# microsoft/Nova

Hardware: NVIDIA H100
Metric: MSM throughput (2^20 BN254 scalar*G1/s) (higher is better)
Workload: dtype u32 limbs (256-bit prime-field / curve integers)

## Files before the change

### nova_b200/csrc/field.cuh

```cuda
#pragma once
#include <cstdint>
#include "field_constants.cuh"

#if defined(__CUDACC__)
#define NOVA_HD __host__ __device__ __forceinline__
#define NOVA_D __device__ __forceinline__
#else
#define NOVA_HD inline
#define NOVA_D inline
#endif

namespace nova {

struct alignas(16) fe_t {
  uint32_t l[8];
};


template <int OFF, bool CIN, int N>
NOVA_HD void chain_mad(uint32_t (&X)[N], uint32_t x0, uint32_t x1, uint32_t x2, uint32_t x3,
                       uint32_t y, uint32_t ca = 0, uint32_t cb = 0) {
  static_assert(OFF + 8 < N, "accumulator too short");
#ifdef __CUDA_ARCH__
  if constexpr (CIN) {
    asm("{\n\t"
        ".reg .u32 t;\n\t"
        "add.cc.u32 t, %14, %15;\n\t"
        "madc.lo.cc.u32 %0, %9, %13, %0;\n\t"
        "madc.hi.cc.u32 %1, %9, %13, %1;\n\t"
        "madc.lo.cc.u32 %2, %10, %13, %2;\n\t"
        "madc.hi.cc.u32 %3, %10, %13, %3;\n\t"
        "madc.lo.cc.u32 %4, %11, %13, %4;\n\t"
        "madc.hi.cc.u32 %5, %11, %13, %5;\n\t"
        "madc.lo.cc.u32 %6, %12, %13, %6;\n\t"
        "madc.hi.cc.u32 %7, %12, %13, %7;\n\t"
        "addc.u32 %8, %8, 0;\n\t"
        "}"
        : "+r"(X[OFF + 0]), "+r"(X[OFF + 1]), "+r"(X[OFF + 2]), "+r"(X[OFF + 3]),
          "+r"(X[OFF + 4]), "+r"(X[OFF + 5]), "+r"(X[OFF + 6]), "+r"(X[OFF + 7]),
          "+r"(X[OFF + 8])
        : "r"(x0), "r"(x1), "r"(x2), "r"(x3), "r"(y), "r"(ca), "r"(cb));
  } else {
    asm("mad.lo.cc.u32 %0, %9, %13, %0;\n\t"
        "madc.hi.cc.u32 %1, %9, %13, %1;\n\t"
        "madc.lo.cc.u32 %2, %10, %13, %2;\n\t"
        "madc.hi.cc.u32 %3, %10, %13, %3;\n\t"
        "madc.lo.cc.u32 %4, %11, %13, %4;\n\t"
        "madc.hi.cc.u32 %5, %11, %13, %5;\n\t"
        "madc.lo.cc.u32 %6, %12, %13, %6;\n\t"
        "madc.hi.cc.u32 %7, %12, %13, %7;\n\t"
        "addc.u32 %8, %8, 0;"
        : "+r"(X[OFF + 0]), "+r"(X[OFF + 1]), "+r"(X[OFF + 2]), "+r"(X[OFF + 3]),
          "+r"(X[OFF + 4]), "+r"(X[OFF + 5]), "+r"(X[OFF + 6]), "+r"(X[OFF + 7]),
          "+r"(X[OFF + 8])
        : "r"(x0), "r"(x1), "r"(x2), "r"(x3), "r"(y));
  }
#else
  uint64_t cf = CIN ? (((uint64_t)ca + cb) >> 32) : 0;
  const uint32_t xs[4] = {x0, x1, x2, x3};
  for (int k = 0; k < 4; k++) {
    uint64_t prod = (uint64_t)xs[k] * y;
    uint64_t t = (uint64_t)X[OFF + 2 * k] + (uint32_t)prod + cf;
    X[OFF + 2 * k] = (uint32_t)t;
    cf = t >> 32;
    t = (uint64_t)X[OFF + 2 * k + 1] + (prod >> 32) + cf;
    X[OFF + 2 * k + 1] = (uint32_t)t;
    cf = t >> 32;
  }
  X[OFF + 8] += (uint32_t)cf;
#endif
}

NOVA_HD void add8(uint32_t (&r)[8], const uint32_t (&a)[8], const uint32_t (&b)[8]) {
#ifdef __CUDA_ARCH__
  asm("add.cc.u32 %0, %8, %16;\n\t"
      "addc.cc.u32 %1, %9, %17;\n\t"
      "addc.cc.u32 %2, %10, %18;\n\t"
      "addc.cc.u32 %3, %11, %19;\n\t"
      "addc.cc.u32 %4, %12, %20;\n\t"
      "addc.cc.u32 %5, %13, %21;\n\t"
      "addc.cc.u32 %6, %14, %22;\n\t"
      "addc.u32 %7, %15, %23;"
      : "=r"(r[0]), "=r"(r[1]), "=r"(r[2]), "=r"(r[3]), "=r"(r[4]), "=r"(r[5]), "=r"(r[6]),
        "=r"(r[7])
      : "r"(a[0]), "r"(a[1]), "r"(a[2]), "r"(a[3]), "r"(a[4]), "r"(a[5]), "r"(a[6]), "r"(a[7]),
        "r"(b[0]), "r"(b[1]), "r"(b[2]), "r"(b[3]), "r"(b[4]), "r"(b[5]), "r"(b[6]), "r"(b[7]));
#else
  uint64_t c = 0;
  for (int i = 0; i < 8; i++) {
    uint64_t t = (uint64_t)a[i] + b[i] + c;
    r[i] = (uint32_t)t;
    c = t >> 32;
  }
#endif
}

NOVA_HD void add8_cin(uint32_t (&r)[8], const uint32_t* a, const uint32_t* b, uint32_t ca,
                      uint32_t cb) {
#ifdef __CUDA_ARCH__
  asm("{\n\t"
      ".reg .u32 t;\n\t"
      "add.cc.u32 t, %24, %25;\n\t"
      "addc.cc.u32 %0, %8, %16;\n\t"
      "addc.cc.u32 %1, %9, %17;\n\t"
      "addc.cc.u32 %2, %10, %18;\n\t"
      "addc.cc.u32 %3, %11, %19;\n\t"
      "addc.cc.u32 %4, %12, %20;\n\t"
      "addc.cc.u32 %5, %13, %21;\n\t"
      "addc.cc.u32 %6, %14, %22;\n\t"
      "addc.u32 %7, %15, %23;\n\t"
      "}"
      : "=r"(r[0]), "=r"(r[1]), "=r"(r[2]), "=r"(r[3]), "=r"(r[4]), "=r"(r[5]), "=r"(r[6]),
        "=r"(r[7])
      : "r"(a[0]), "r"(a[1]), "r"(a[2]), "r"(a[3]), "r"(a[4]), "r"(a[5]), "r"(a[6]), "r"(a[7]),
        "r"(b[0]), "r"(b[1]), "r"(b[2]), "r"(b[3]), "r"(b[4]), "r"(b[5]), "r"(b[6]), "r"(b[7]),
        "r"(ca), "r"(cb));
#else
  uint64_t c = ((uint64_t)ca + cb) >> 32;
  for (int i = 0; i < 8; i++) {
    uint64_t t = (uint64_t)a[i] + b[i] + c;
    r[i] = (uint32_t)t;
    c = t >> 32;
  }
#endif
}

NOVA_HD uint32_t sub8(uint32_t (&r)[8], const uint32_t (&a)[8], const uint32_t (&b)[8]) {
  uint32_t borrow;
#ifdef __CUDA_ARCH__
  asm("sub.cc.u32 %0, %9, %17;\n\t"
      "subc.cc.u32 %1, %10, %18;\n\t"
      "subc.cc.u32 %2, %11, %19;\n\t"
      "subc.cc.u32 %3, %12, %20;\n\t"
      "subc.cc.u32 %4, %13, %21;\n\t"
      "subc.cc.u32 %5, %14, %22;\n\t"
      "subc.cc.u32 %6, %15, %23;\n\t"
      "subc.cc.u32 %7, %16, %24;\n\t"
      "subc.u32 %8, 0, 0;"
      : "=r"(r[0]), "=r"(r[1]), "=r"(r[2]), "=r"(r[3]), "=r"(r[4]), "=r"(r[5]), "=r"(r[6]),
        "=r"(r[7]), "=r"(borrow)
      : "r"(a[0]), "r"(a[1]), "r"(a[2]), "r"(a[3]), "r"(a[4]), "r"(a[5]), "r"(a[6]), "r"(a[7]),
        "r"(b[0]), "r"(b[1]), "r"(b[2]), "r"(b[3]), "r"(b[4]), "r"(b[5]), "r"(b[6]), "r"(b[7]));
#else
  uint64_t c = 0;
  for (int i = 0; i < 8; i++) {
    uint64_t t = (uint64_t)a[i] - b[i] - c;
    r[i] = (uint32_t)t;
    c = (t >> 32) & 1;
  }
  borrow = c ? 0xffffffffu : 0u;
#endif
  return borrow;
}

template <class F>
NOVA_HD void load_p(uint32_t (&p)[8]) {
#pragma unroll
  for (int i = 0; i < 8; i++) p[i] = F::p(i);
}


template <class F>
NOVA_HD fe_t fe_zero() {
  fe_t r;
#pragma unroll
  for (int i = 0; i < 8; i++) r.l[i] = 0;
  return r;
}

template <class F>
NOVA_HD fe_t fe_one() {
  fe_t r;
#pragma unroll
  for (int i = 0; i < 8; i++) r.l[i] = F::r(i);
  return r;
}

NOVA_HD bool fe_is_zero(const fe_t& a) {
  return (a.l[0] | a.l[1] | a.l[2] | a.l[3] | a.l[4] | a.l[5] | a.l[6] | a.l[7]) == 0;
}

NOVA_HD bool fe_eq(const fe_t& a, const fe_t& b) {
  return ((a.l[0] ^ b.l[0]) | (a.l[1] ^ b.l[1]) | (a.l[2] ^ b.l[2]) | (a.l[3] ^ b.l[3]) |
          (a.l[4] ^ b.l[4]) | (a.l[5] ^ b.l[5]) | (a.l[6] ^ b.l[6]) | (a.l[7] ^ b.l[7])) == 0;
}

template <class F>
NOVA_HD bool fe_is_canonical(const fe_t& a) {
  uint32_t p[8], t[8];
  load_p<F>(p);
  return sub8(t, a.l, p) != 0;
}

template <class F>
NOVA_HD void fe_reduce_once(uint32_t (&r)[8]) {
  uint32_t p[8], t[8];
  load_p<F>(p);
  uint32_t borrow = sub8(t, r, p);
#pragma unroll
  for (int i = 0; i < 8; i++) r[i] = borrow ? r[i] : t[i];
}

template <class F>
NOVA_HD fe_t fe_add(const fe_t& a, const fe_t& b) {
  fe_t r;
  add8(r.l, a.l, b.l);
  fe_reduce_once<F>(r.l);
  return r;
}

template <class F>
NOVA_HD fe_t fe_sub(const fe_t& a, const fe_t& b) {
  fe_t r;
  uint32_t p[8], t[8];
  load_p<F>(p);
  uint32_t borrow = sub8(r.l, a.l, b.l);
  add8(t, r.l, p);
#pragma unroll
  for (int i = 0; i < 8; i++) r.l[i] = borrow ? t[i] : r.l[i];
  return r;
}

template <class F>
NOVA_HD fe_t fe_neg(const fe_t& a) {
  fe_t z = fe_zero<F>();
  return fe_is_zero(a) ? z : fe_sub<F>(z, a);
}

template <class F>
NOVA_HD fe_t fe_dbl(const fe_t& a) {
  return fe_add<F>(a, a);
}

template <class F, int I>
NOVA_HD void mont_round(uint32_t (&E)[17], uint32_t (&O)[17], const fe_t& a, uint32_t bi) {
  if constexpr ((I & 1) == 0) {
    if constexpr (I == 0)
      chain_mad<I, false>(E, a.l[0], a.l[2], a.l[4], a.l[6], bi);
    else
      chain_mad<I, true>(E, a.l[0], a.l[2], a.l[4], a.l[6], bi, E[I - 1], O[I - 1]);
    chain_mad<I + 1, false>(O, a.l[1], a.l[3], a.l[5], a.l[7], bi);
    uint32_t m = (E[I] + O[I]) * F::INV;
    chain_mad<I, false>(E, F::p(0), F::p(2), F::p(4), F::p(6), m);
    chain_mad<I + 1, false>(O, F::p(1), F::p(3), F::p(5), F::p(7), m);
  } else {
    chain_mad<I, true>(O, a.l[0], a.l[2], a.l[4], a.l[6], bi, E[I - 1], O[I - 1]);
    chain_mad<I + 1, false>(E, a.l[1], a.l[3], a.l[5], a.l[7], bi);
    uint32_t m = (E[I] + O[I]) * F::INV;
    chain_mad<I, false>(O, F::p(0), F::p(2), F::p(4), F::p(6), m);
    chain_mad<I + 1, false>(E, F::p(1), F::p(3), F::p(5), F::p(7), m);
  }
}

template <class F>
NOVA_HD fe_t fe_mul_chain(const fe_t& a, const fe_t& b) {
  uint32_t E[17], O[17];
#pragma unroll
  for (int i = 0; i < 17; i++) E[i] = O[i] = 0;
  mont_round<F, 0>(E, O, a, b.l[0]);
  mont_round<F, 1>(E, O, a, b.l[1]);
  mont_round<F, 2>(E, O, a, b.l[2]);
  mont_round<F, 3>(E, O, a, b.l[3]);
  mont_round<F, 4>(E, O, a, b.l[4]);
  mont_round<F, 5>(E, O, a, b.l[5]);
  mont_round<F, 6>(E, O, a, b.l[6]);
  mont_round<F, 7>(E, O, a, b.l[7]);
  fe_t r;
  add8_cin(r.l, &E[8], &O[8], E[7], O[7]);
  fe_reduce_once<F>(r.l);
  return r;
}

template <class F, int I>
NOVA_HD void mont_round2(uint32_t (&E)[17], uint32_t (&O)[17], const fe_t& a, uint32_t bi, const fe_t& c,
                         uint32_t di) {
  if constexpr ((I & 1) == 0) {
    if constexpr (I == 0)
      chain_mad<I, false>(E, a.l[0], a.l[2], a.l[4], a.l[6], bi);
    else
      chain_mad<I, true>(E, a.l[0], a.l[2], a.l[4], a.l[6], bi, E[I - 1], O[I - 1]);
    chain_mad<I + 1, false>(O, a.l[1], a.l[3], a.l[5], a.l[7], bi);
    chain_mad<I, false>(E, c.l[0], c.l[2], c.l[4], c.l[6], di);
    chain_mad<I + 1, false>(O, c.l[1], c.l[3], c.l[5], c.l[7], di);
    uint32_t m = (E[I] + O[I]) * F::INV;
    chain_mad<I, false>(E, F::p(0), F::p(2), F::p(4), F::p(6), m);
    chain_mad<I + 1, false>(O, F::p(1), F::p(3), F::p(5), F::p(7), m);
  } else {
    chain_mad<I, true>(O, a.l[0], a.l[2], a.l[4], a.l[6], bi, E[I - 1], O[I - 1]);
    chain_mad<I + 1, false>(E, a.l[1], a.l[3], a.l[5], a.l[7], bi);
    chain_mad<I, false>(O, c.l[0], c.l[2], c.l[4], c.l[6], di);
    chain_mad<I + 1, false>(E, c.l[1], c.l[3], c.l[5], c.l[7], di);
    uint32_t m = (E[I] + O[I]) * F::INV;
    chain_mad<I, false>(O, F::p(0), F::p(2), F::p(4), F::p(6), m);
    chain_mad<I + 1, false>(E, F::p(1), F::p(3), F::p(5), F::p(7), m);
  }
}

template <class F>
NOVA_HD fe_t fe_mul2_add(const fe_t& a, const fe_t& b, const fe_t& c, const fe_t& d) {
  uint32_t E[17], O[17];
#pragma unroll
  for (int i = 0; i < 17; i++) E[i] = O[i] = 0;
  mont_round2<F, 0>(E, O, a, b.l[0], c, d.l[0]);
  mont_round2<F, 1>(E, O, a, b.l[1], c, d.l[1]);
  mont_round2<F, 2>(E, O, a, b.l[2], c, d.l[2]);
  mont_round2<F, 3>(E, O, a, b.l[3], c, d.l[3]);
  mont_round2<F, 4>(E, O, a, b.l[4], c, d.l[4]);
  mont_round2<F, 5>(E, O, a, b.l[5], c, d.l[5]);
  mont_round2<F, 6>(E, O, a, b.l[6], c, d.l[6]);
  mont_round2<F, 7>(E, O, a, b.l[7], c, d.l[7]);
  fe_t r;
  add8_cin(r.l, &E[8], &O[8], E[7], O[7]);
  fe_reduce_once<F>(r.l);
  return r;
}

NOVA_HD void mad_cs(uint32_t& lo, uint32_t& hi, uint32_t& k, uint32_t x, uint32_t y) {
#ifdef __CUDA_ARCH__
  asm("mad.lo.cc.u32 %0, %3, %4, %0;\n\t"
      "madc.hi.cc.u32 %1, %3, %4, %1;\n\t"
      "addc.u32 %2, %2, 0;"
      : "+r"(lo), "+r"(hi), "+r"(k)
      : "r"(x), "r"(y));
#else
  uint64_t acc = ((uint64_t)hi << 32) | lo;
  uint64_t prod = (uint64_t)x * y;
  uint64_t s = acc + prod;
  k += s < prod ? 1u : 0u;
  lo = (uint32_t)s;
  hi = (uint32_t)(s >> 32);
#endif
}

NOVA_HD void retire_cs(uint32_t& k_next, uint32_t e, uint32_t o, uint32_t kz) {
#ifdef __CUDA_ARCH__
  [[maybe_unused]] uint32_t t;
  asm("add.cc.u32 %1, %2, %3;\n\t"
      "addc.u32 %0, %0, %4;"
      : "+r"(k_next), "=r"(t)
      : "r"(e), "r"(o), "r"(kz));
#else
  k_next += (uint32_t)(((uint64_t)e + o) >> 32) + kz;
#endif
}

template <class F, int I>
NOVA_HD void mont_round_cs(uint32_t (&E)[16], uint32_t (&O)[16], uint32_t (&K)[17], const fe_t& a,
                           uint32_t bi) {
  uint32_t(&A)[16] = (I & 1) ? O : E;
  uint32_t(&B)[16] = (I & 1) ? E : O;
  mad_cs(A[I + 0], A[I + 1], K[I + 2], a.l[0], bi);
  mad_cs(B[I + 1], B[I + 2], K[I + 3], a.l[1], bi);
  mad_cs(A[I + 2], A[I + 3], K[I + 4], a.l[2], bi);
  mad_cs(B[I + 3], B[I + 4], K[I + 5], a.l[3], bi);
  mad_cs(A[I + 4], A[I + 5], K[I + 6], a.l[4], bi);
  mad_cs(B[I + 5], B[I + 6], K[I + 7], a.l[5], bi);
  mad_cs(A[I + 6], A[I + 7], K[I + 8], a.l[6], bi);
  mad_cs(B[I + 7], B[I + 8], K[I + 9], a.l[7], bi);
  uint32_t m = (E[I] + O[I] + K[I]) * F::INV;
  mad_cs(A[I + 0], A[I + 1], K[I + 2], F::p(0), m);
  mad_cs(B[I + 1], B[I + 2], K[I + 3], F::p(1), m);
  mad_cs(A[I + 2], A[I + 3], K[I + 4], F::p(2), m);
  mad_cs(B[I + 3], B[I + 4], K[I + 5], F::p(3), m);
  mad_cs(A[I + 4], A[I + 5], K[I + 6], F::p(4), m);
  mad_cs(B[I + 5], B[I + 6], K[I + 7], F::p(5), m);
  mad_cs(A[I + 6], A[I + 7], K[I + 8], F::p(6), m);
  mad_cs(B[I + 7], B[I + 8], K[I + 9], F::p(7), m);
  retire_cs(K[I + 1], E[I], O[I], K[I] ? 1u : 0u);
}

template <class F>
NOVA_HD fe_t fe_mul_cs(const fe_t& a, const fe_t& b) {
  uint32_t E[16], O[16], K[17];
#pragma unroll
  for (int i = 0; i < 16; i++) E[i] = O[i] = K[i] = 0;
  K[16] = 0;
  mont_round_cs<F, 0>(E, O, K, a, b.l[0]);
  mont_round_cs<F, 1>(E, O, K, a, b.l[1]);
  mont_round_cs<F, 2>(E, O, K, a, b.l[2]);
  mont_round_cs<F, 3>(E, O, K, a, b.l[3]);
  mont_round_cs<F, 4>(E, O, K, a, b.l[4]);
  mont_round_cs<F, 5>(E, O, K, a, b.l[5]);
  mont_round_cs<F, 6>(E, O, K, a, b.l[6]);
  mont_round_cs<F, 7>(E, O, K, a, b.l[7]);
  uint32_t hiE[8], hiO[8], hiK[8], t[8];
#pragma unroll
  for (int i = 0; i < 8; i++) {
    hiE[i] = E[8 + i];
    hiO[i] = O[8 + i];
    hiK[i] = K[8 + i];
  }
  fe_t r;
  add8(t, hiE, hiO);
  add8(r.l, t, hiK);
  fe_reduce_once<F>(r.l);
  return r;
}

template <class F>
NOVA_HD fe_t fe_mul(const fe_t& a, const fe_t& b) {
#ifdef NOVA_MUL_CS
  return fe_mul_cs<F>(a, b);
#else
  return fe_mul_chain<F>(a, b);
#endif
}


template <int OFF, int NP, int N>
NOVA_HD void chain_mad_n(uint32_t (&X)[N], uint32_t x0, uint32_t x1, uint32_t x2, uint32_t x3, uint32_t y) {
  static_assert(NP >= 1 && NP <= 4 && OFF + 2 * NP < N, "chain does not fit the accumulator");
#ifdef __CUDA_ARCH__
  if constexpr (NP == 1) {
    asm("mad.lo.cc.u32 %0, %3, %4, %0;\n\t"
        "madc.hi.cc.u32 %1, %3, %4, %1;\n\t"
        "addc.u32 %2, %2, 0;"
        : "+r"(X[OFF + 0]), "+r"(X[OFF + 1]), "+r"(X[OFF + 2])
        : "r"(x0), "r"(y));
  } else if constexpr (NP == 2) {
    asm("mad.lo.cc.u32 %0, %5, %7, %0;\n\t"
        "madc.hi.cc.u32 %1, %5, %7, %1;\n\t"
        "madc.lo.cc.u32 %2, %6, %7, %2;\n\t"
        "madc.hi.cc.u32 %3, %6, %7, %3;\n\t"
        "addc.u32 %4, %4, 0;"
        : "+r"(X[OFF + 0]), "+r"(X[OFF + 1]), "+r"(X[OFF + 2]), "+r"(X[OFF + 3]), "+r"(X[OFF + 4])
        : "r"(x0), "r"(x1), "r"(y));
  } else if constexpr (NP == 3) {
    asm("mad.lo.cc.u32 %0, %7, %10, %0;\n\t"
        "madc.hi.cc.u32 %1, %7, %10, %1;\n\t"
        "madc.lo.cc.u32 %2, %8, %10, %2;\n\t"
        "madc.hi.cc.u32 %3, %8, %10, %3;\n\t"
        "madc.lo.cc.u32 %4, %9, %10, %4;\n\t"
        "madc.hi.cc.u32 %5, %9, %10, %5;\n\t"
        "addc.u32 %6, %6, 0;"
        : "+r"(X[OFF + 0]), "+r"(X[OFF + 1]), "+r"(X[OFF + 2]), "+r"(X[OFF + 3]), "+r"(X[OFF + 4]),
          "+r"(X[OFF + 5]), "+r"(X[OFF + 6])
        : "r"(x0), "r"(x1), "r"(x2), "r"(y));
  } else {
    asm("mad.lo.cc.u32 %0, %9, %13, %0;\n\t"
        "madc.hi.cc.u32 %1, %9, %13, %1;\n\t"
        "madc.lo.cc.u32 %2, %10, %13, %2;\n\t"
        "madc.hi.cc.u32 %3, %10, %13, %3;\n\t"
        "madc.lo.cc.u32 %4, %11, %13, %4;\n\t"
        "madc.hi.cc.u32 %5, %11, %13, %5;\n\t"
        "madc.lo.cc.u32 %6, %12, %13, %6;\n\t"
        "madc.hi.cc.u32 %7, %12, %13, %7;\n\t"
        "addc.u32 %8, %8, 0;"
        : "+r"(X[OFF + 0]), "+r"(X[OFF + 1]), "+r"(X[OFF + 2]), "+r"(X[OFF + 3]), "+r"(X[OFF + 4]),
          "+r"(X[OFF + 5]), "+r"(X[OFF + 6]), "+r"(X[OFF + 7]), "+r"(X[OFF + 8])
        : "r"(x0), "r"(x1), "r"(x2), "r"(x3), "r"(y));
  }
#else
  const uint32_t xs[4] = {x0, x1, x2, x3};
  uint64_t cf = 0;
  for (int k = 0; k < NP; k++) {
    uint64_t prod = (uint64_t)xs[k] * y;
    uint64_t t = (uint64_t)X[OFF + 2 * k] + (uint32_t)prod + cf;
    X[OFF + 2 * k] = (uint32_t)t;
    cf = t >> 32;
    t = (uint64_t)X[OFF + 2 * k + 1] + (prod >> 32) + cf;
    X[OFF + 2 * k + 1] = (uint32_t)t;
    cf = t >> 32;
  }
  X[OFF + 2 * NP] += (uint32_t)cf;
#endif
}

NOVA_HD void chain_sqr_diag(uint32_t (&X)[17], const fe_t& a) {
#ifdef __CUDA_ARCH__
  asm("mad.lo.cc.u32 %0, %17, %17, %0;\n\t"
      "madc.hi.cc.u32 %1, %17, %17, %1;\n\t"
      "madc.lo.cc.u32 %2, %18, %18, %2;\n\t"
      "madc.hi.cc.u32 %3, %18, %18, %3;\n\t"
      "madc.lo.cc.u32 %4, %19, %19, %4;\n\t"
      "madc.hi.cc.u32 %5, %19, %19, %5;\n\t"
      "madc.lo.cc.u32 %6, %20, %20, %6;\n\t"
      "madc.hi.cc.u32 %7, %20, %20, %7;\n\t"
      "madc.lo.cc.u32 %8, %21, %21, %8;\n\t"
      "madc.hi.cc.u32 %9, %21, %21, %9;\n\t"
      "madc.lo.cc.u32 %10, %22, %22, %10;\n\t"
      "madc.hi.cc.u32 %11, %22, %22, %11;\n\t"
      "madc.lo.cc.u32 %12, %23, %23, %12;\n\t"
      "madc.hi.cc.u32 %13, %23, %23, %13;\n\t"
      "madc.lo.cc.u32 %14, %24, %24, %14;\n\t"
      "madc.hi.cc.u32 %15, %24, %24, %15;\n\t"
      "addc.u32 %16, %16, 0;"
      : "+r"(X[0]), "+r"(X[1]), "+r"(X[2]), "+r"(X[3]), "+r"(X[4]), "+r"(X[5]), "+r"(X[6]), "+r"(X[7]),
        "+r"(X[8]), "+r"(X[9]), "+r"(X[10]), "+r"(X[11]), "+r"(X[12]), "+r"(X[13]), "+r"(X[14]), "+r"(X[15]),
        "+r"(X[16])
      : "r"(a.l[0]), "r"(a.l[1]), "r"(a.l[2]), "r"(a.l[3]), "r"(a.l[4]), "r"(a.l[5]), "r"(a.l[6]), "r"(a.l[7]));
#else
  uint64_t cf = 0;
  for (int k = 0; k < 8; k++) {
    uint64_t prod = (uint64_t)a.l[k] * a.l[k];
    uint64_t t = (uint64_t)X[2 * k] + (uint32_t)prod + cf;
    X[2 * k] = (uint32_t)t;
    cf = t >> 32;
    t = (uint64_t)X[2 * k + 1] + (prod >> 32) + cf;
    X[2 * k + 1] = (uint32_t)t;
    cf = t >> 32;
  }
  X[16] += (uint32_t)cf;
#endif
}

template <int J>
NOVA_HD void sqr_cross(uint32_t (&E)[17], uint32_t (&O)[17], const fe_t& a) {
  constexpr int SAME0 = J & 1;
  constexpr int NSAME = J / 2;
  constexpr int OTH0 = 1 - (J & 1);
  constexpr int NOTH = (J + 1) / 2;
  const uint32_t y = a.l[J];
  auto limb = [&](int i) { return i < 8 ? a.l[i] : 0u; };
  if constexpr (NSAME > 0)
    chain_mad_n<SAME0 + J, NSAME>(E, limb(SAME0), limb(SAME0 + 2), limb(SAME0 + 4), limb(SAME0 + 6), y);
  if constexpr (NOTH > 0)
    chain_mad_n<OTH0 + J, NOTH>(O, limb(OTH0), limb(OTH0 + 2), limb(OTH0 + 4), limb(OTH0 + 6), y);
}

template <class F, int I>
NOVA_HD void mont_reduce_round(uint32_t (&E)[17], uint32_t (&O)[17]) {
  uint32_t c = 0;
  if constexpr (I > 0) c = (uint32_t)(((uint64_t)E[I - 1] + O[I - 1]) >> 32);
  const uint32_t m = (E[I] + O[I] + c) * F::INV;
  if constexpr ((I & 1) == 0) {
    if constexpr (I == 0)
      chain_mad<I, false>(E, F::p(0), F::p(2), F::p(4), F::p(6), m);
    else
      chain_mad<I, true>(E, F::p(0), F::p(2), F::p(4), F::p(6), m, E[I - 1], O[I - 1]);
    chain_mad<I + 1, false>(O, F::p(1), F::p(3), F::p(5), F::p(7), m);
  } else {
    chain_mad<I, true>(O, F::p(0), F::p(2), F::p(4), F::p(6), m, E[I - 1], O[I - 1]);
    chain_mad<I + 1, false>(E, F::p(1), F::p(3), F::p(5), F::p(7), m);
  }
}

template <class F>
NOVA_HD fe_t fe_sqr_dedicated(const fe_t& a) {
  uint32_t E[17], O[17];
#pragma unroll
  for (int i = 0; i < 17; i++) E[i] = O[i] = 0;
  sqr_cross<1>(E, O, a);
  sqr_cross<2>(E, O, a);
  sqr_cross<3>(E, O, a);
  sqr_cross<4>(E, O, a);
  sqr_cross<5>(E, O, a);
  sqr_cross<6>(E, O, a);
  sqr_cross<7>(E, O, a);
#pragma unroll
  for (int i = 16; i > 0; i--) {
    E[i] = (E[i] << 1) | (E[i - 1] >> 31);
    O[i] = (O[i] << 1) | (O[i - 1] >> 31);
  }
  E[0] <<= 1;
  O[0] <<= 1;
  chain_sqr_diag(E, a);
  uint32_t hiE[8], hiO[8], lo[8], hi[8];
#pragma unroll
  for (int i = 0; i < 8; i++) {
    hiE[i] = E[8 + i];
    hiO[i] = O[8 + i];
    E[8 + i] = 0;
    O[8 + i] = 0;
  }
  E[16] = O[16] = 0;
  mont_reduce_round<F, 0>(E, O);
  mont_reduce_round<F, 1>(E, O);
  mont_reduce_round<F, 2>(E, O);
  mont_reduce_round<F, 3>(E, O);
  mont_reduce_round<F, 4>(E, O);
  mont_reduce_round<F, 5>(E, O);
  mont_reduce_round<F, 6>(E, O);
  mont_reduce_round<F, 7>(E, O);
  add8_cin(lo, &E[8], &O[8], E[7], O[7]);
  add8(hi, hiE, hiO);
  fe_t r;
  add8(r.l, hi, lo);
  fe_reduce_once<F>(r.l);
  return r;
}

template <class F>
NOVA_HD fe_t fe_sqr(const fe_t& a) {
#if defined(NOVA_SQR_DEDICATED) && !defined(NOVA_MUL_CS)
  return fe_sqr_dedicated<F>(a);
#else
  return fe_mul<F>(a, a);
#endif
}

template <class F>
NOVA_HD fe_t fe_from_mont(const fe_t& a) {
  fe_t one;
#pragma unroll
  for (int i = 0; i < 8; i++) one.l[i] = (i == 0);
  return fe_mul<F>(a, one);
}

template <class F>
NOVA_HD fe_t fe_to_mont(const fe_t& a) {
  fe_t r2;
#pragma unroll
  for (int i = 0; i < 8; i++) r2.l[i] = F::r2(i);
  return fe_mul<F>(a, r2);
}

template <class F>
NOVA_HD fe_t fe_inv(const fe_t& a) {
  uint32_t e[8];
  uint32_t bw = 2;
#pragma unroll
  for (int i = 0; i < 8; i++) {
    uint32_t pi = F::p(i);
    e[i] = pi - bw;
    bw = (pi < bw) ? 1u : 0u;
  }
  fe_t acc = fe_one<F>();
  for (int i = 255; i >= 0; i--) {
    acc = fe_sqr<F>(acc);
    if ((e[i >> 5] >> (i & 31)) & 1) acc = fe_mul<F>(acc, a);
  }
  return acc;
}

#if defined(__CUDACC__)
NOVA_D fe_t fe_load(const void* base, size_t idx) {
  const uint4* p = reinterpret_cast<const uint4*>(base) + 2 * idx;
  uint4 lo = __ldg(p), hi = __ldg(p + 1);
  fe_t r;
  r.l[0] = lo.x; r.l[1] = lo.y; r.l[2] = lo.z; r.l[3] = lo.w;
  r.l[4] = hi.x; r.l[5] = hi.y; r.l[6] = hi.z; r.l[7] = hi.w;
  return r;
}
NOVA_D fe_t fe_load_rw(const void* base, size_t idx) {
  const uint4* p = reinterpret_cast<const uint4*>(base) + 2 * idx;
  uint4 lo = p[0], hi = p[1];
  fe_t r;
  r.l[0] = lo.x; r.l[1] = lo.y; r.l[2] = lo.z; r.l[3] = lo.w;
  r.l[4] = hi.x; r.l[5] = hi.y; r.l[6] = hi.z; r.l[7] = hi.w;
  return r;
}
NOVA_D void fe_store(void* base, size_t idx, const fe_t& a) {
  uint4* p = reinterpret_cast<uint4*>(base) + 2 * idx;
  p[0] = make_uint4(a.l[0], a.l[1], a.l[2], a.l[3]);
  p[1] = make_uint4(a.l[4], a.l[5], a.l[6], a.l[7]);
}
#elif defined(NOVA_SIMT_HOST)
inline fe_t fe_load(const void* base, size_t idx) { return reinterpret_cast<const fe_t*>(base)[idx]; }
inline fe_t fe_load_rw(const void* base, size_t idx) { return reinterpret_cast<const fe_t*>(base)[idx]; }
inline void fe_store(void* base, size_t idx, const fe_t& a) { reinterpret_cast<fe_t*>(base)[idx] = a; }
#endif

}
```

### nova_b200/csrc/msm_sort.cuh

```cuda
#pragma once
#if !defined(NOVA_SIMT_HOST)
#include <cuda_runtime.h>
#endif
#include <cstddef>
#include <cstdint>
#include "field.cuh"

namespace nova {

constexpr uint32_t NO_KEY = 0xFFFFFFFFu;

constexpr int SORT_THREADS = 256;
constexpr int SORT_WARPS = SORT_THREADS / 32;
constexpr int SORT_ITEMS = 16;
constexpr int SORT_TILE = SORT_THREADS * SORT_ITEMS;
constexpr int SORT_RADIX_MAX = 8;
constexpr int SORT_BINS = 1 << SORT_RADIX_MAX;
constexpr int SORT_PASSES_MAX = 4;
constexpr int SORT_CTL_WORDS = SORT_PASSES_MAX * SORT_BINS + SORT_PASSES_MAX;
constexpr unsigned SORT_HIST_BLOCKS = 1024;
constexpr int SORT_LOOK_WINDOW = 4;
constexpr int SORT_MIN_BLOCKS = 3;
static_assert(SORT_BINS == SORT_THREADS, "the per-bin steps run one bin per thread");

struct sort_plan {
  int passes;
  int bits;
};

inline sort_plan make_sort_plan(uint64_t K) {
  int kb = 1;
  while (kb < 32 && ((uint64_t)1 << kb) < K) kb++;
  sort_plan sp;
  sp.passes = (kb + SORT_RADIX_MAX - 1) / SORT_RADIX_MAX;
  sp.bits = (kb + sp.passes - 1) / sp.passes;
  return sp;
}

struct sort_args {
  uint32_t n;
  uint32_t count;
  int W, G;
  uint32_t B;
  uint32_t n_ck;
  uint32_t base_offset;
  uint32_t blind_i;
  uint32_t h_index;
  sort_plan sp;
};

NOVA_D void sort_hist_clear(uint32_t* sh ) {
  for (int i = threadIdx.x; i < SORT_PASSES_MAX * SORT_BINS; i += blockDim.x) sh[i] = 0;
  __syncthreads();
}

NOVA_D void sort_hist_count(uint32_t* sh, uint32_t key, const sort_plan sp) {
  const bool live = key != NO_KEY;
  const unsigned live_mask = __ballot_sync(0xFFFFFFFFu, live);
  if (live_mask == 0) return;
  const unsigned lane = threadIdx.x & 31u, leader = (unsigned)(__ffs(live_mask) - 1);
  const uint32_t lead_key = __shfl_sync(0xFFFFFFFFu, key, (int)leader);
  const bool same = __ballot_sync(0xFFFFFFFFu, live && key != lead_key) == 0;
  const uint32_t mask = (1u << sp.bits) - 1;
  for (int p = 0; p < sp.passes; p++) {
    const uint32_t bin = (key >> (p * sp.bits)) & mask;
    if (same) {
      if (lane == leader) atomicAdd(&sh[p * SORT_BINS + bin], (uint32_t)__popc(live_mask));
    } else if (live) {
      atomicAdd(&sh[p * SORT_BINS + bin], 1u);
    }
  }
}

NOVA_D void sort_hist_flush(const uint32_t* sh, uint32_t* hist, const sort_plan sp) {
  __syncthreads();
  for (int i = threadIdx.x; i < sp.passes * SORT_BINS; i += blockDim.x) {
    const uint32_t v = sh[i];
    if (v) atomicAdd(&hist[i], v);
  }
}

static __global__ void __launch_bounds__(256) k_digits_small(const void* __restrict__ scalars, int elem_bytes,
                                                             size_t n, int c, int W, int G, uint32_t B,
                                                             int32_t* __restrict__ digits, uint32_t* __restrict__ hist,
                                                             const sort_plan sp) {
  __shared__ uint32_t s_hist[SORT_PASSES_MAX * SORT_BINS];
  sort_hist_clear(s_hist);
  for (size_t blk = (size_t)blockIdx.x * blockDim.x; blk < n; blk += (size_t)gridDim.x * blockDim.x) {
    const size_t i = blk + threadIdx.x;
    const bool live = i < n;
    uint64_t v64 = 0;
    if (live) switch (elem_bytes) {
      case 1: v64 = ((const uint8_t*)scalars)[i]; break;
      case 2: v64 = ((const uint16_t*)scalars)[i]; break;
      case 4: v64 = ((const uint32_t*)scalars)[i]; break;
      default: v64 = ((const uint64_t*)scalars)[i]; break;
    }
    const uint32_t half = 1u << (c - 1);
    const uint64_t mask = (1ull << c) - 1;
    uint32_t carry = 0;
    for (int w = 0; w < W; w++) {
      int bit = w * c;
      uint32_t v = bit < 64 ? (uint32_t)((v64 >> bit) & mask) : 0u;
      v += carry;
      int32_t dgt;
      if (v > half) {
        dgt = (int32_t)v - (int32_t)(1u << c);
        carry = 1;
      } else {
        dgt = (int32_t)v;
        carry = 0;
      }
      if (live) digits[(size_t)w * n + i] = dgt;
      uint32_t key = NO_KEY;
      if (dgt != 0) {
        uint32_t mag = dgt < 0 ? (uint32_t)(-dgt) : (uint32_t)dgt;
        key = (uint32_t)(w % G) * B + (mag - 1);
      }
      sort_hist_count(s_hist, key, sp);
    }
  }
  sort_hist_flush(s_hist, hist, sp);
}

NOVA_D uint32_t sort_block_scan(uint32_t v, uint32_t* s_tmp, uint32_t* total) {
  const int lane = threadIdx.x & 31, warp = threadIdx.x >> 5;
  uint32_t inc = v;
#pragma unroll
  for (int d = 1; d < 32; d <<= 1) {
    const uint32_t o = __shfl_up_sync(0xFFFFFFFFu, inc, d);
    if (lane >= d) inc += o;
  }
  if (lane == 31) s_tmp[warp] = inc;
  __syncthreads();
  uint32_t before = 0, all = 0;
#pragma unroll
  for (int w = 0; w < SORT_WARPS; w++) {
    const uint32_t t = s_tmp[w];
    before += w < warp ? t : 0u;
    all += t;
  }
  __syncthreads();
  *total = all;
  return before + inc - v;
}

constexpr unsigned long long LOOK_INCLUSIVE = 1ull << 32;
NOVA_D unsigned long long look_word(uint32_t tag, bool inclusive, uint32_t v) {
  return ((unsigned long long)tag << 33) | (inclusive ? LOOK_INCLUSIVE : 0ull) | v;
}

template <bool FIRST>
__global__ void __launch_bounds__(SORT_THREADS, SORT_MIN_BLOCKS) k_sort_pass(const int32_t* __restrict__ digits,
                                                            const uint64_t* __restrict__ in,
                                                            uint64_t* __restrict__ out, const sort_args a, int pass,
                                                            uint32_t* __restrict__ ctl,
                                                            unsigned long long* __restrict__ look, uint32_t tag) {
  __shared__ uint64_t s_items[SORT_TILE];
  __shared__ uint32_t s_warp[SORT_WARPS][SORT_BINS];
  __shared__ uint32_t s_glob[SORT_BINS];
  __shared__ uint32_t s_tmp[SORT_WARPS];
  __shared__ uint32_t s_tile;
  const int tid = threadIdx.x, lane = tid & 31, warp = tid >> 5;
  const unsigned lt_mask = (1u << lane) - 1u;
  const int shift = pass * a.sp.bits;
  const uint32_t mask = (1u << a.sp.bits) - 1u;

  if (tid == 0) s_tile = atomicAdd(&ctl[SORT_PASSES_MAX * SORT_BINS + pass], 1u);
#pragma unroll
  for (int w = 0; w < SORT_WARPS; w++) s_warp[w][tid] = 0;
  uint32_t M;
  const uint32_t bin_base = sort_block_scan(ctl[pass * SORT_BINS + tid], s_tmp, &M);
  const uint32_t tile = s_tile;
  const uint32_t count = FIRST ? a.count : M;
  if ((uint64_t)tile * SORT_TILE >= count) return;
  const uint32_t wbase = tile * SORT_TILE + warp * 32 * SORT_ITEMS + lane;

  uint64_t item[SORT_ITEMS];
#pragma unroll
  for (int j = 0; j < SORT_ITEMS; j++) {
    const uint32_t idx = wbase + 32u * j;
    if (FIRST) item[j] = idx < count ? (uint64_t)(uint32_t)digits[idx] : 0ull;
    else item[j] = idx < count ? in[idx] : 0ull;
  }
  uint32_t rank[SORT_ITEMS];
#pragma unroll
  for (int j = 0; j < SORT_ITEMS; j++) {
    const uint32_t idx = wbase + 32u * j;
    bool valid;
    if (FIRST) {
      const int32_t dgt = (int32_t)(uint32_t)item[j];
      valid = idx < count && dgt != 0;
      if (valid) {
        const uint32_t w = idx / a.n, i = idx - w * a.n;
        const uint32_t sign = dgt < 0 ? 1u : 0u;
        const uint32_t mag = sign ? (uint32_t)(-dgt) : (uint32_t)dgt;
        const uint32_t key = (w % (uint32_t)a.G) * a.B + (mag - 1);
        const uint32_t bi = i == a.blind_i ? a.h_index : a.base_offset + i;
        const uint32_t tix = (w / (uint32_t)a.G) * a.n_ck + bi;
        item[j] = ((uint64_t)key << 32) | ((uint64_t)sign << 31) | tix;
      }
    } else {
      valid = idx < count;
    }
    const uint32_t bin = (uint32_t)(item[j] >> (32 + shift)) & mask;
    unsigned peers = __ballot_sync(0xFFFFFFFFu, valid);
    rank[j] = NO_KEY;
    if (peers) {
      for (int b = 0; b < a.sp.bits; b++) {
        const unsigned m = __ballot_sync(0xFFFFFFFFu, (bin >> b) & 1u);
        peers &= ((bin >> b) & 1u) ? m : ~m;
      }
      const uint32_t before = valid ? s_warp[warp][bin] : 0u;
      __syncwarp();
      if (valid) {
        rank[j] = before + (uint32_t)__popc(peers & lt_mask);
        if ((peers & lt_mask) == 0) s_warp[warp][bin] = before + (uint32_t)__popc(peers);
      }
      __syncwarp();
    }
  }
  __syncthreads();

  uint32_t run = 0;
#pragma unroll
  for (int w = 0; w < SORT_WARPS; w++) {
    const uint32_t c = s_warp[w][tid];
    s_warp[w][tid] = run;
    run += c;
  }
  volatile unsigned long long* vlook = look;
  const size_t slot = (size_t)tile * SORT_BINS + tid;
  vlook[slot] = look_word(tag, tile == 0, run);
  uint32_t tile_total;
  const uint32_t tile_off = sort_block_scan(run, s_tmp, &tile_total);
  uint32_t excl = 0;
  for (uint32_t t = tile; t > 0;) {
    unsigned long long v[SORT_LOOK_WINDOW];
#pragma unroll
    for (int q = 0; q < SORT_LOOK_WINDOW; q++)
      v[q] = (uint32_t)q < t ? vlook[(size_t)(t - 1 - q) * SORT_BINS + tid] : 0ull;
    bool go = true;
#pragma unroll
    for (int q = 0; q < SORT_LOOK_WINDOW; q++) {
      go = go && t > 0 && (uint32_t)(v[q] >> 33) == tag;
      if (go) {
        excl += (uint32_t)v[q];
        t = (v[q] & LOOK_INCLUSIVE) ? 0u : t - 1;
      }
    }
  }
  if (tile != 0) vlook[slot] = look_word(tag, true, excl + run);
  s_glob[tid] = bin_base + excl - tile_off;
#pragma unroll
  for (int w = 0; w < SORT_WARPS; w++) s_warp[w][tid] += tile_off;
  __syncthreads();

#pragma unroll
  for (int j = 0; j < SORT_ITEMS; j++) {
    if (rank[j] != NO_KEY) {
      const uint32_t bin = (uint32_t)(item[j] >> (32 + shift)) & mask;
      s_items[s_warp[warp][bin] + rank[j]] = item[j];
    }
  }
  __syncthreads();
  for (uint32_t k = tid; k < tile_total; k += SORT_THREADS) {
    const uint64_t e = s_items[k];
    const uint32_t bin = (uint32_t)(e >> (32 + shift)) & mask;
    out[s_glob[bin] + k] = e;
  }
}

static __global__ void __launch_bounds__(SORT_THREADS) k_sort_starts(const uint64_t* __restrict__ entries,
                                                              const uint32_t* __restrict__ ctl, const sort_plan sp,
                                                              uint32_t K, uint32_t* __restrict__ start,
                                                              uint32_t* __restrict__ heavy, uint32_t heavy_min,
                                                              uint32_t heavy_cap) {
  __shared__ uint32_t s_base[SORT_BINS + 1];
  __shared__ uint32_t s_start[SORT_THREADS + 1];
  __shared__ uint32_t s_tmp[SORT_WARPS];
  const int tid = threadIdx.x;
  const int last = sp.passes - 1, shift = last * sp.bits;
  uint32_t M;
  s_base[tid] = sort_block_scan(ctl[last * SORT_BINS + tid], s_tmp, &M);
  if (tid == 0) s_base[SORT_BINS] = M;
  __syncthreads();
  auto lower_bound = [&](uint32_t k) -> uint32_t {
    if (k >= K) return M;
    const uint32_t top = k >> shift;
    uint32_t lo = s_base[top], hi = s_base[top + 1];
    while (lo < hi) {
      const uint32_t mid = lo + (hi - lo) / 2;
      if ((uint32_t)(entries[mid] >> 32) < k) lo = mid + 1;
      else hi = mid;
    }
    return lo;
  };
  const uint32_t k = blockIdx.x * SORT_THREADS + tid;
  s_start[tid] = lower_bound(k);
  if (tid == SORT_THREADS - 1) s_start[SORT_THREADS] = lower_bound(k + 1);
  __syncthreads();
  if (k <= K) start[k] = s_start[tid];
  if (k < K && s_start[tid + 1] - s_start[tid] > heavy_min) {
    const uint32_t slot = atomicAdd(&heavy[0], 1u);
    if (slot < heavy_cap) heavy[1 + slot] = k;
  }
}

}
```

Baseline: 274.9 million.

## Specialize from-Montgomery reduction, raise histogram blocks, strength-reduce sort index division

fe_from_mont now runs eight Montgomery reduction rounds on the input directly instead of a full multiplication by one, removing the partial-product work. The sort histogram grid grows from 1024 to 4096 blocks. In the first scatter pass, the per-item window/group/index division and modulo are replaced by incremental counters advanced by 32 per item, which avoids integer divisions per key. The counter update loop handles the case where n is smaller than 32 by looping, adding branches.

```diff
diff --git a/nova_b200/csrc/field.cuh b/nova_b200/csrc/field.cuh
--- a/nova_b200/csrc/field.cuh
+++ b/nova_b200/csrc/field.cuh
@@ -591,10 +591,23 @@
 
 template <class F>
 NOVA_HD fe_t fe_from_mont(const fe_t& a) {
-  fe_t one;
-#pragma unroll
-  for (int i = 0; i < 8; i++) one.l[i] = (i == 0);
-  return fe_mul<F>(a, one);
+  uint32_t E[17], O[17];
+#pragma unroll
+  for (int i = 0; i < 17; i++) E[i] = O[i] = 0;
+#pragma unroll
+  for (int i = 0; i < 8; i++) E[i] = a.l[i];
+  mont_reduce_round<F, 0>(E, O);
+  mont_reduce_round<F, 1>(E, O);
+  mont_reduce_round<F, 2>(E, O);
+  mont_reduce_round<F, 3>(E, O);
+  mont_reduce_round<F, 4>(E, O);
+  mont_reduce_round<F, 5>(E, O);
+  mont_reduce_round<F, 6>(E, O);
+  mont_reduce_round<F, 7>(E, O);
+  fe_t r;
+  add8_cin(r.l, &E[8], &O[8], E[7], O[7]);
+  fe_reduce_once<F>(r.l);
+  return r;
 }
 
 template <class F>
diff --git a/nova_b200/csrc/msm_sort.cuh b/nova_b200/csrc/msm_sort.cuh
--- a/nova_b200/csrc/msm_sort.cuh
+++ b/nova_b200/csrc/msm_sort.cuh
@@ -18,7 +18,7 @@
 constexpr int SORT_BINS = 1 << SORT_RADIX_MAX;
 constexpr int SORT_PASSES_MAX = 4;
 constexpr int SORT_CTL_WORDS = SORT_PASSES_MAX * SORT_BINS + SORT_PASSES_MAX;
-constexpr unsigned SORT_HIST_BLOCKS = 1024;
+constexpr unsigned SORT_HIST_BLOCKS = 4096;
 constexpr int SORT_LOOK_WINDOW = 4;
 constexpr int SORT_MIN_BLOCKS = 3;
 static_assert(SORT_BINS == SORT_THREADS, "the per-bin steps run one bin per thread");
@@ -184,20 +184,32 @@
     else item[j] = idx < count ? in[idx] : 0ull;
   }
   uint32_t rank[SORT_ITEMS];
+  uint32_t i = 0, g = 0, t = 0;
+  if (FIRST) {
+    const uint32_t w = wbase / a.n;
+    i = wbase - w * a.n;
+    t = w / (uint32_t)a.G;
+    g = w - t * (uint32_t)a.G;
+  }
 #pragma unroll
   for (int j = 0; j < SORT_ITEMS; j++) {
     const uint32_t idx = wbase + 32u * j;
     bool valid;
     if (FIRST) {
+      if (j)
+        for (i += 32; i >= a.n; i -= a.n)
+          if (++g == (uint32_t)a.G) {
+            g = 0;
+            t++;
+          }
       const int32_t dgt = (int32_t)(uint32_t)item[j];
       valid = idx < count && dgt != 0;
       if (valid) {
-        const uint32_t w = idx / a.n, i = idx - w * a.n;
         const uint32_t sign = dgt < 0 ? 1u : 0u;
         const uint32_t mag = sign ? (uint32_t)(-dgt) : (uint32_t)dgt;
-        const uint32_t key = (w % (uint32_t)a.G) * a.B + (mag - 1);
+        const uint32_t key = g * a.B + (mag - 1);
         const uint32_t bi = i == a.blind_i ? a.h_index : a.base_offset + i;
-        const uint32_t tix = (w / (uint32_t)a.G) * a.n_ck + bi;
+        const uint32_t tix = t * a.n_ck + bi;
         item[j] = ((uint64_t)key << 32) | ((uint64_t)sign << 31) | tix;
       }
     } else {
```

After: 278.5 million, median of 6. 1.01x the previous value.
